# Roywangj/AdaptPoint

Measured on AMD Instinct MI355X. Metric: set-abstraction fwd+bwd point-clouds/sec (B=32,N=1024), higher is better.
Workload: dtype bf16

## Files before the change

### adaptpoint_amd/csrc/sa_fused.hip

```cpp
#include "apn_common.h"
#include "apn_mfma.h"
#include <type_traits>
#include "sa_chain.h"

namespace apn {

constexpr int SA_C = 32;
constexpr int SA_C1 = 32;
constexpr int SA_C2 = 64;
constexpr int SA_K = 32;
constexpr int SA_WAVES = 4;

template <int NS>
__device__ __forceinline__ void put_frag(uint4 *base, int f, int lane, const Frag<NS> &v) {
#pragma unroll
    for (int p = 0; p < NS; ++p) base[(f * NS + p) * 64 + lane] = __builtin_bit_cast(uint4, v.p[p]);
}

template <int NS>
__device__ __forceinline__ Frag<NS> get_frag(const uint4 *base, int f, int lane) {
    Frag<NS> v;
#pragma unroll
    for (int p = 0; p < NS; ++p) v.p[p] = __builtin_bit_cast(bf16x8, base[(f * NS + p) * 64 + lane]);
    return v;
// ... 292 lines not shown
    int nst = 3;
    for (; tile < tiles; slot += stride, tile = remap(slot)) {
        const bool more = remap(slot + stride) < tiles;
        const int tile2 = remap(slot + 2 * stride);
        if (LATE) {
            const TileHead hd_nxt2 = load_head<CP>(a, tile2 < tiles ? tile2 : tile, r);
            body(tile, cur, nst == 4, [&] {
                asm volatile("" ::: "memory");
                touch(hd_nxt);
                if (more) {
                    ahead(hd_nxt);
                    fetch_tile<NS>(a, hd_nxt, h, cur);
                }
            });
            stamp(a, wave, nst < 5 ? nst : 5);
            ++nst;
            hd_nxt = hd_nxt2;
            continue;
        }
        touch(hd_nxt);
        pre();
        if (more) fetch_tile<NS>(a, hd_nxt, h, nxt);
        const TileHead hd_nxt2 = load_head<CP>(a, tile2 < tiles ? tile2 : tile, r);
        body(tile, cur, nst == 4, [&] { touch(hd_nxt2); });
        stamp(a, wave, nst < 5 ? nst : 5);
        ++nst;
        if (more) cur = nxt;
        hd_nxt = hd_nxt2;
    }
    pre();
    stamp(a, wave, 6);
}

template <int NV>
__device__ __forceinline__ float fold_partials(float (&vals)[NV], int lane, int wave) {
    __shared__ float red[SA_WAVES][NV][32];
#pragma unroll
    for (int i = 0; i < NV; ++i) {
        const float other = __shfl_xor(vals[i], 32);
        if (lane < 32) red[wave][i][lane] = vals[i] + other;
    }
    __syncthreads();
    float s = 0.0f;
    const int e = threadIdx.x;
    if (e < NV * 32) {
#pragma unroll
        for (int w = 0; w < SA_WAVES; ++w) s += red[w][e >> 5][e & 31];
    }
    return s;
}

__device__ __forceinline__ void fold_rows32(const float *__restrict__ part, int rows, const double *__restrict__ sums,
                                            const BnArgs &bn, float *__restrict__ pack, float &scale, float &shift,
                                            double *scratch ) {
    double (*fred)[64] = reinterpret_cast<double (*)[64]>(scratch);
    double *ftot = scratch + 16 * 64;
    const int tid = threadIdx.x;
    double count = bn.count;
    double gpre = 1.0, bpre = 0.0;
    if (tid < 32) {
        if (bn.gamma) gpre = (double)bn.gamma[tid];
        if (bn.beta) bpre = (double)bn.beta[tid];
    }
    if (bn.training) {
        if (part) {
            const int quad = tid & 15, rg = tid >> 4;
            const float4 *__restrict__ p4 = reinterpret_cast<const float4 *>(part) + quad;
            double s0 = 0.0, s1 = 0.0, s2 = 0.0, s3 = 0.0;
            int rr = rg;
            for (; rr + 7 * 16 < rows; rr += 8 * 16) {
                float4 v[8];
#pragma unroll
                for (int u = 0; u < 8; ++u) v[u] = p4[(size_t)(rr + 16 * u) * 16];
#pragma unroll
                for (int u = 0; u < 8; ++u) {
                    s0 += (double)v[u].x; s1 += (double)v[u].y; s2 += (double)v[u].z; s3 += (double)v[u].w;
                }
            }
            for (; rr + 3 * 16 < rows; rr += 4 * 16) {
                float4 v[4];
#pragma unroll
                for (int u = 0; u < 4; ++u) v[u] = p4[(size_t)(rr + 16 * u) * 16];
#pragma unroll
                for (int u = 0; u < 4; ++u) {
                    s0 += (double)v[u].x; s1 += (double)v[u].y; s2 += (double)v[u].z; s3 += (double)v[u].w;
                }
            }
            for (; rr < rows; rr += 16) {
                const float4 v = p4[(size_t)rr * 16];
                s0 += (double)v.x; s1 += (double)v.y; s2 += (double)v.z; s3 += (double)v.w;
            }
            fred[rg][4 * quad] = s0; fred[rg][4 * quad + 1] = s1; fred[rg][4 * quad + 2] = s2; fred[rg][4 * quad + 3] = s3;
            __syncthreads();
            if (tid < 64) {
                double s = 0.0;
#pragma unroll
                for (int k = 0; k < 16; ++k) s += fred[k][tid];
                ftot[tid] = s;
            }
        } else if (tid < 64) {
            ftot[tid] = sums[tid];
        }
        if (!part) count = sums[64];
        __syncthreads();
    }
    if (tid < 32) {
        if (tid == 0 && blockIdx.x == 0 && bn.training && bn.nbt) *bn.nbt += 1;
        bn_channel(bn, 32, tid, bn.training ? ftot[tid] : 0.0, bn.training ? ftot[32 + tid] : 0.0, count,
                   blockIdx.x == 0, pack, scale, shift, gpre, bpre);
    }
}

template <int NS, bool CP>
__global__ __launch_bounds__(SA_WAVES * 64, 3) void sa_fwd_main_kernel(
    SaArgs a, const float *__restrict__ w2, BnArgs bn1, const float *__restrict__ part1, int rows1,
    const double *__restrict__ sums1, float *__restrict__ pack1, const float *__restrict__ gamma2,
    float *__restrict__ ysel, unsigned char *__restrict__ ksel, unsigned long long *__restrict__ acc2) {
    const int lane = threadIdx.x & 63, r = lane & 31, h = lane >> 5;
    const int wave = __builtin_amdgcn_readfirstlane(threadIdx.x >> 6);
    enum { F_W1 = 0, F_W2 = 3, F_COUNT = 7 };
    __shared__ uint4 cfrag[F_COUNT * NS * 64];
    __shared__ __attribute__((aligned(16))) float bn1v[2][2][16];
    constexpr int PT_WAVE = CP ? 2 * 32 * 33 : 17 * 64 * 2 / SA_WAVES;
    __shared__ __attribute__((aligned(16))) float ptile[SA_WAVES * PT_WAVE];
    __shared__ __attribute__((aligned(16))) unsigned sinfo[SA_WAVES][32];
    static_assert(SA_WAVES * PT_WAVE * 4 >= 17 * 64 * 8, "fold scratch");
    critical_stream_priority();
    stamp(a, wave, 0);
    const float sg[2] = {(!gamma2 || gamma2[r] >= 0.0f) ? 1.0f : -1.0f, (!gamma2 || gamma2[32 + r] >= 0.0f) ? 1.0f : -1.0f};
    float st[4] = {0.0f, 0.0f, 0.0f, 0.0f};

    auto prologue = [&]() {
        if (wave == 0) {
            Frag<NS> w1f[3];
            load_w1_frags<NS>(a.w1, r, h, w1f);
#pragma unroll
            for (int s = 0; s < 3; ++s) put_frag<NS>(cfrag, F_W1 + s, lane, w1f[s]);
        }
        if (wave == 1 || wave == 2) {
            const int t = wave - 1;
#pragma unroll
            for (int s = 0; s < 2; ++s) {
                float tmp[8];
#pragma unroll
                for (int j = 0; j < 8; ++j) tmp[j] = w2[(32 * t + r) * SA_C1 + acc_row(8 * s + j, h)];
                put_frag<NS>(cfrag, F_W2 + 2 * t + s, lane, make_frag<NS>(tmp));
            }
        }
        float sc, sh;
        fold_rows32(part1, rows1, sums1, bn1, pack1, sc, sh, reinterpret_cast<double *>(ptile));
        if (threadIdx.x < 32) {
            const int i = threadIdx.x;
            bn1v[0][(i >> 2) & 1][(i & 3) + 4 * (i >> 3)] = sc;
            bn1v[1][(i >> 2) & 1][(i & 3) + 4 * (i >> 3)] = sh;
        }
        __syncthreads();
    };

    for_each_tile<NS, CP>(a, wave, r, h, prologue, [] {}, [&](int tile, const TileRaw<NS> &raw, bool, auto before_stores) {
        int lane_o = lane;
        asm volatile("" : "+v"(lane_o));
        Frag<NS> x[3];
        build_frags<NS>(a, raw, h, x);
        const int q0 = __builtin_amdgcn_readfirstlane(raw.q0);
        const int nq = __builtin_amdgcn_readfirstlane((int)(raw.info >> 24));
        float multf[16];
        unsigned starts = 1u;
        float *pt = ptile + wave * PT_WAVE;
        if (CP) {
            if (lane < 32) sinfo[wave][lane] = raw.info;
#pragma unroll
            for (int gq = 0; gq < 4; ++gq) {
                const uint4 v = *reinterpret_cast<const uint4 *>(&sinfo[wave][8 * gq + 4 * (lane_o >> 5)]);
                multf[4 * gq] = (float)ri_mult(v.x); multf[4 * gq + 1] = (float)ri_mult(v.y);
                multf[4 * gq + 2] = (float)ri_mult(v.z); multf[4 * gq + 3] = (float)ri_mult(v.w);
            }
            const unsigned prev = (unsigned)__shfl_up((int)raw.info, 1);
            starts = (unsigned)__ballot(lane < 32 && (lane == 0 || ri_q(raw.info) != ri_q(prev)));
        }
        f32x16 y1 = {0};
#pragma unroll
        for (int s = 0; s < 3; ++s) y1 = mfma<NS>(get_frag<NS>(cfrag, F_W1 + s, lane_o), x[s], y1);
        {
            const float4 *scv = reinterpret_cast<const float4 *>(bn1v[0][lane_o >> 5]);
            const float4 *shv = reinterpret_cast<const float4 *>(bn1v[1][lane_o >> 5]);
#pragma unroll
            for (int i4 = 0; i4 < 4; ++i4) {
                const float4 sc = scv[i4], sh = shv[i4];
                y1[4 * i4] = __builtin_fmaxf(__builtin_fmaf(y1[4 * i4], sc.x, sh.x), 0.0f);
                y1[4 * i4 + 1] = __builtin_fmaxf(__builtin_fmaf(y1[4 * i4 + 1], sc.y, sh.y), 0.0f);
                y1[4 * i4 + 2] = __builtin_fmaxf(__builtin_fmaf(y1[4 * i4 + 2], sc.z, sh.z), 0.0f);
                y1[4 * i4 + 3] = __builtin_fmaxf(__builtin_fmaf(y1[4 * i4 + 3], sc.w, sh.w), 0.0f);
            }
        }
        const Frag<NS> a0 = pack8<NS>(y1, 0), a1 = pack8<NS>(y1, 8);
#pragma unroll
        for (int t = 0; t < 2; ++t) {
            f32x16 y2 = {0};
            y2 = mfma<NS>(a0, get_frag<NS>(cfrag, F_W2 + 2 * t, lane_o), y2);
            y2 = mfma<NS>(a1, get_frag<NS>(cfrag, F_W2 + 2 * t + 1, lane_o), y2);
            if (CP) {
                float s1 = 0.0f, s2 = 0.0f;
#pragma unroll
                for (int i = 0; i < 16; ++i) {
                    const float wy = multf[i] * y2[i];
                    s1 += wy;
                    s2 += wy * y2[i];
                    pt[(t * 32 + acc_row(i, h)) * 33 + r] = sg[t] * y2[i];
                }
                st[t] += s1;
                st[2 + t] += s2;
                continue;
            }
            float best = sg[t] * y2[0];
            int bpos = 0;
            float s1 = 0.0f, s2 = 0.0f;
#pragma unroll
            for (int i = 0; i < 16; ++i) {
                s1 += y2[i];
                s2 += y2[i] * y2[i];
                const float v = sg[t] * y2[i];
                if (i > 0 && v > best) { best = v; bpos = i; }
            }
            st[t] += s1;
            st[2 + t] += s2;
            int kpos = acc_row(bpos, h);
            const float obest = __shfl_xor(best, 32);
            const int okpos = __shfl_xor(kpos, 32);
            if (obest > best || (obest == best && okpos < kpos)) { best = obest; kpos = okpos; }
            if (h == 0) {
                ysel[(size_t)tile * SA_C2 + 32 * t + r] = sg[t] * best;
                ksel[(size_t)tile * SA_C2 + 32 * t + r] = (unsigned char)kpos;
            }
        }
        if (CP) {
            asm volatile("" ::: "memory");
            const float *mine = pt + h * (32 * 33) + r;
            const float sgn = h ? sg[1] : sg[0];
            float *ys = ysel + (size_t)q0 * SA_C2 + lane;
            unsigned char *ks = ksel + (size_t)q0 * SA_C2 + lane;
            before_stores();
            int seg = -1, ra = 0, kpos = 0;
            float best = 0.0f;
#pragma unroll
            for (int half16 = 0; half16 < 2; ++half16) {
                float v[16];
#pragma unroll
                for (int i = 0; i < 16; ++i) v[i] = mine[(16 * half16 + i) * 33];
#pragma unroll
                for (int i = 0; i < 16; ++i) {
                    const int rho = 16 * half16 + i;
                    if ((starts >> rho) & 1u) {
                        if (seg >= 0 && seg < nq) {
                            ys[(size_t)seg * SA_C2] = sgn * best;
                            ks[(size_t)seg * SA_C2] = (unsigned char)kpos;
                        }
                        ++seg;
                        best = -__builtin_inff();
                        kpos = 0;
                        ra = rho;
                    }
                    const bool up = v[i] > best;
                    best = up ? v[i] : best;
                    kpos = up ? rho - ra : kpos;
                }
            }
            if (seg >= 0 && seg < nq) {
                ys[(size_t)seg * SA_C2] = sgn * best;
                ks[(size_t)seg * SA_C2] = (unsigned char)kpos;
            }
            asm volatile("" ::: "memory");
        }
    });
    const float tot = fold_partials<4>(st, lane, wave);
    if (threadIdx.x < 128) acc_add(acc2, 128, blockIdx.x % ACC_COPIES, threadIdx.x, tot);
    stamp(a, wave, 7);
}

struct SaBwdArgs {
    const float *w2;
    const float *scale1, *shift1, *mean1, *inv1;
    const float *pack2;
    const unsigned long long *accS;
    const double *sumsS;
    double count;
    int train2;
    const float *goa;
    const unsigned char *ksel;
    const int *rowdst;
};

template <int NS, bool CP>
__global__ __launch_bounds__(SA_WAVES * 64, 2) void sa_bwd_kernel(SaArgs a, SaBwdArgs g,
                                                               unsigned long long *__restrict__ accT,
                                                               float *__restrict__ partW2,
                                                               float *__restrict__ GU,
                                                               float *__restrict__ HA,
                                                               float *__restrict__ HB) {
    static_assert(CP, "the backward pass runs over a tile map");
    const int lane = threadIdx.x & 63, r = lane & 31, h = lane >> 5;
    const int wave = __builtin_amdgcn_readfirstlane(threadIdx.x >> 6);
    enum { F_W1 = 0, F_QM = 3, F_W2T = 5, F_COUNT = 9 };
    __shared__ uint4 cfrag[F_COUNT * NS * 64];
    __shared__ __attribute__((aligned(16))) float bn1v[2][2][16];
    __shared__ __attribute__((aligned(16))) float sw2[SA_C2][SA_C1 + 4];
    __shared__ float sD[SA_C2], sE[SA_C2];
    __shared__ __attribute__((aligned(16))) float sqm[SA_C1 + 1][SA_C1 + 4];
    critical_stream_priority();
    stamp(a, wave, 0);
    __shared__ float chan[5][32];
    f32x16 dsp[2] = {{0}, {0}};
    f32x16 gram = {0};
    float suma = 0.0f;
    float st[2] = {0.0f, 0.0f};

    constexpr int SP_ROW = 72, SP_TILE = 32 * SP_ROW;
    constexpr int SP_WAVE = (CP && NS * SP_TILE * 2 < 2 * 32 * 33 * 4) ? 2 * 32 * 33 * 4 : NS * SP_TILE * 2;
    constexpr int SP_BYTES = SA_WAVES * SP_WAVE, WRED_BYTES = SA_WAVES * SA_C2 * SA_C1 * 4;
    __shared__ __attribute__((aligned(16))) unsigned char sp_raw[SP_BYTES > WRED_BYTES ? SP_BYTES : WRED_BYTES];
    __shared__ __attribute__((aligned(16))) unsigned sinfo[SA_WAVES][32];
    __shared__ __attribute__((aligned(16))) float qgoa[CP ? SA_WAVES : 1][4 * SA_C2];
    __shared__ __attribute__((aligned(16))) unsigned char qksel[CP ? SA_WAVES : 1][4 * SA_C2];
    __bf16 *sp_img = reinterpret_cast<__bf16 *>(sp_raw + wave * SP_WAVE);

    __shared__ __attribute__((aligned(16))) int sdst[SA_WAVES][2][64];
    int ahead_n = 0, body_n = 0;
    auto gu_store = [&](int place, float v) {
        *reinterpret_cast<float *>(reinterpret_cast<char *>(GU) + (((unsigned)place << 7) + ((unsigned)r << 2))) = v;
    };

    auto prologue = [&]() {
        const int tid = threadIdx.x;
        {
            Frag<NS> w1f[3];
            if (wave == 0) load_w1_frags<NS>(a.w1, r, h, w1f);
            float wv[8];
#pragma unroll
            for (int k = 0; k < 8; ++k) wv[k] = g.w2[tid + 256 * k];
            float c1[4] = {0.f, 0.f, 0.f, 0.f};
            if (tid >= 128 && tid < 160) {
                c1[0] = g.scale1[tid - 128]; c1[1] = g.shift1[tid - 128]; c1[2] = g.mean1[tid - 128]; c1[3] = g.inv1[tid - 128];
            }
            double sv = 0.0, count = g.count;
            float p_sc = 0.0f, p_mu = 0.0f, p_iv = 0.0f;
            if (tid < 128) sv = g.sumsS ? g.sumsS[tid] : acc_read(g.accS, 128, tid);
            if (g.sumsS) count = g.sumsS[128];
            if (tid < 64) { p_sc = g.pack2[tid]; p_mu = g.pack2[128 + tid]; p_iv = g.pack2[192 + tid]; }
            if (wave == 0) {
#pragma unroll
                for (int s = 0; s < 3; ++s) put_frag<NS>(cfrag, F_W1 + s, lane, w1f[s]);
            }
#pragma unroll
            for (int k = 0; k < 8; ++k) sw2[(tid + 256 * k) >> 5][tid & 31] = wv[k];
            if (tid >= 128 && tid < 160) {
#pragma unroll
                for (int k = 0; k < 4; ++k) chan[k][tid - 128] = c1[k];
            }
            double *sS2 = reinterpret_cast<double *>(&sqm[0][0]);
            if (tid >= 64 && tid < 128) sS2[tid - 64] = sv;
            __syncthreads();
            if (tid < 64) {
                const double sc = p_sc, mu = p_mu, iv = p_iv, s1 = sv, s2 = sS2[tid];
                double d = 0.0, e = 0.0;
                if (g.train2) {
                    const double rc = 1.0 / count;
                    d = -sc * iv * s2 * rc;
                    e = (-sc * s1 + sc * mu * iv * s2) * rc;
                }
                sD[tid] = (float)d;
                sE[tid] = (float)e;
            }
            if (tid >= 64 && tid < 96) {
                const int i = tid - 64;
                const float sci = g.scale1[i], shi = g.shift1[i];
                bn1v[0][(i >> 2) & 1][(i & 3) + 4 * (i >> 3)] = sci;
                bn1v[1][(i >> 2) & 1][(i & 3) + 4 * (i >> 3)] = shi;
            }
        }
        __syncthreads();
        {
            const int s = wave;
            float tmp[8], tmpd[8], tmpe[8];
#pragma unroll
            for (int j = 0; j < 8; ++j) {
                const int c = 16 * s + 8 * h + j;
                tmp[j] = sw2[c][r];
                tmpd[j] = tmp[j] * sD[c];
                tmpe[j] = r == 0 ? sE[c] : 0.0f;
            }
            const Frag<NS> wt = make_frag<NS>(tmp);
            put_frag<NS>(cfrag, F_W2T + s, lane, wt);
            const f32x16 zero16 = {0};
            const f32x16 qp = mfma<NS>(make_frag<NS>(tmpd), wt, zero16);
            const f32x16 ep = mfma<NS>(make_frag<NS>(tmpe), wt, zero16);
            float *scr = reinterpret_cast<float *>(sp_img);
#pragma unroll
            for (int e = 0; e < 16; ++e) scr[e * 64 + lane] = qp[e];
            if (h == 0) scr[16 * 64 + r] = ep[0];
        }
        __syncthreads();
        if (wave == 2) {
            f32x16 qacc = {0};
            float ev = 0.0f;
#pragma unroll
            for (int w = 0; w < SA_WAVES; ++w) {
                const float *pw = reinterpret_cast<const float *>(sp_raw + w * SP_WAVE);
#pragma unroll
                for (int e = 0; e < 16; ++e) qacc[e] += pw[e * 64 + lane];
                if (h == 0) ev += pw[16 * 64 + r];
            }
            put_frag<NS>(cfrag, F_QM, lane, pack8<NS>(qacc, 0));
            put_frag<NS>(cfrag, F_QM + 1, lane, pack8<NS>(qacc, 8));
            if (h == 0) chan[4][r] = ev;
        }
        __syncthreads();
        {
            uint4 *z = reinterpret_cast<uint4 *>(sp_img);
            for (int e = lane; e < SP_WAVE / 16; e += 64) z[e] = make_uint4(0u, 0u, 0u, 0u);
        }
    };

    auto scatter_pending = [] {};
    auto ahead = [&](const TileHead &hd) {
        if (!CP) return;
        typedef __attribute__((address_space(3))) void lds_void;
        typedef __attribute__((address_space(1))) const void glb_void;
        const int q0n = __builtin_amdgcn_readfirstlane(hd.q0);
        const int qbn = q0n < a.b * a.m - 4 ? q0n : a.b * a.m - 4;
        int l_o = lane;
        asm volatile("" : "+v"(l_o));
        const char *gb = reinterpret_cast<const char *>(g.goa) + (size_t)qbn * (SA_C2 * 4);
        const char *kb = reinterpret_cast<const char *>(g.ksel) + (size_t)qbn * SA_C2;
        __builtin_amdgcn_global_load_lds((glb_void *)(gb + (unsigned)(16 * l_o)), (lds_void *)&qgoa[wave][0], 16, 0, 0);
        __builtin_amdgcn_global_load_lds((glb_void *)(kb + (unsigned)(4 * l_o)), (lds_void *)&qksel[wave][0], 4, 0, 0);
        const char *db = reinterpret_cast<const char *>(g.rowdst) + (size_t)__builtin_amdgcn_readfirstlane(hd.tile) * (SA_K * 4);
        __builtin_amdgcn_global_load_lds((glb_void *)(db + (unsigned)(4 * (l_o & 31))), (lds_void *)&sdst[wave][ahead_n & 1][0], 4, 0, 0);
        ++ahead_n;
    };
    for_each_tile<NS, CP, CP>(a, wave, r, h, prologue, scatter_pending, [&](int tile, const TileRaw<NS> &raw, bool probe, auto before_stores) {
        auto st2 = [&](int k) { if (probe) stamp(a, wave, 8 + k); };
        st2(0);
        int lane_o = lane;
        asm volatile("" : "+v"(lane_o));
        Frag<NS> x[3];
        build_frags<NS>(a, raw, h, x);

        const int q0 = __builtin_amdgcn_readfirstlane(raw.q0);
        const int nq = CP ? __builtin_amdgcn_readfirstlane((int)(raw.info >> 24)) : 1;
        const bool live_row = !CP || ri_mult(raw.info) != 0;
        const float mrow = CP ? (float)ri_mult(raw.info) : 1.0f;
        float gv4[4];
        int kc4[4];
        const int qb = q0 < a.b * a.m - 4 ? q0 : a.b * a.m - 4;
#pragma unroll
        for (int u = 0; u < 4; ++u) {
            if (CP) {
                gv4[u] = 0.0f;
                kc4[u] = 0;
            } else {
                gv4[u] = 0.0f;
                kc4[u] = 0;
                if (u == 0) {
                    gv4[u] = g.goa[(size_t)(q0 + u) * SA_C2 + lane];
                    kc4[u] = g.ksel[(size_t)(q0 + u) * SA_C2 + lane];
                }
            }
        }
        unsigned mpk[4] = {0x01010101u, 0x01010101u, 0x01010101u, 0x01010101u};
        unsigned starts = 1u;
        if (CP) {
            if (lane < 32) sinfo[wave][lane] = raw.info;
#pragma unroll
            for (int gq = 0; gq < 4; ++gq) {
                const uint4 v = *reinterpret_cast<const uint4 *>(&sinfo[wave][8 * gq + 4 * (lane_o >> 5)]);
                mpk[gq] = ri_mult(v.x) | (ri_mult(v.y) << 8) | (ri_mult(v.z) << 16) | (ri_mult(v.w) << 24);
            }
            const unsigned prev = (unsigned)__shfl_up((int)raw.info, 1);
            starts = (unsigned)__ballot(lane < 32 && (lane == 0 || ri_q(raw.info) != ri_q(prev)));
        }
        auto multf = [&](int i) { return (float)((mpk[i >> 2] >> (8 * (i & 3))) & 0xffu); };
        f32x16 yT = {0}, y1 = {0};
#pragma unroll
        for (int s = 0; s < 3; ++s) {
            const Frag<NS> w = get_frag<NS>(cfrag, F_W1 + s, lane_o);
            yT = mfma<NS>(w, x[s], yT);
            y1 = mfma<NS>(x[s], w, y1);
        }
        {
            const float4 *scv = reinterpret_cast<const float4 *>(bn1v[0][lane_o >> 5]);
            const float4 *shv = reinterpret_cast<const float4 *>(bn1v[1][lane_o >> 5]);
#pragma unroll
            for (int i4 = 0; i4 < 4; ++i4) {
                const float4 sc = scv[i4], sh = shv[i4];
                yT[4 * i4] = __builtin_fmaxf(__builtin_fmaf(yT[4 * i4], sc.x, sh.x), 0.0f);
                yT[4 * i4 + 1] = __builtin_fmaxf(__builtin_fmaf(yT[4 * i4 + 1], sc.y, sh.y), 0.0f);
                yT[4 * i4 + 2] = __builtin_fmaxf(__builtin_fmaf(yT[4 * i4 + 2], sc.z, sh.z), 0.0f);
                yT[4 * i4 + 3] = __builtin_fmaxf(__builtin_fmaf(yT[4 * i4 + 3], sc.w, sh.w), 0.0f);
            }
        }
        st2(1);
        Frag<NS> a0, a1;
        if (CP) {
            f32x16 yw;
#pragma unroll
            for (int i = 0; i < 16; ++i) yw[i] = yT[i] * mrow;
            a0 = pack8<NS>(yw, 0);
            a1 = pack8<NS>(yw, 8);
        } else {
            a0 = pack8<NS>(yT, 0);
            a1 = pack8<NS>(yT, 8);
        }

        Frag<NS> sp[4];
        {
            unsigned todo = starts;
            if (CP) {
                asm volatile("s_waitcnt vmcnt(0)" ::: "memory");
                const int dq = q0 - qb;
#pragma unroll
                for (int u = 0; u < 4; ++u) {
                    const int e = (u + dq < 4 ? u + dq : 3) * SA_C2 + lane_o;
                    gv4[u] = qgoa[wave][e];
                    kc4[u] = qksel[wave][e];
                }
            }
#pragma unroll 1
            for (int jb = 0; jb < nq; jb += 4) {
                if (jb) {
#pragma unroll
                    for (int u = 0; u < 4; ++u)
                        if (jb + u < nq) {
                            gv4[u] = g.goa[(size_t)(q0 + jb + u) * SA_C2 + lane];
                            kc4[u] = g.ksel[(size_t)(q0 + jb + u) * SA_C2 + lane];
                        }
                }
#pragma unroll
                for (int u = 0; u < 4; ++u) {
                    if (jb + u < nq) {
                        const float gv = gv4[u];
                        int kc = kc4[u];
                        if (CP) {
                            kc += __builtin_ctz(todo);
                            todo &= todo - 1u;
                        }
                        const __bf16 ghi = (__bf16)gv;
                        const __bf16 glo = (__bf16)(gv - (float)ghi);
                        __bf16 *cell = sp_img + kc * SP_ROW + lane;
                        cell[0] = ghi;
                        if (NS == 2) cell[SP_TILE] = glo;
                        if (!CP) kc4[u] = kc;
                    }
                }
            }
        }
        asm volatile("" ::: "memory");
        {
            f32x16 an;
            const float sc1 = chan[0][lane_o & 31], sh1 = chan[1][lane_o & 31];
#pragma unroll
            for (int i = 0; i < 16; ++i) {
                an[i] = __builtin_fmaxf(__builtin_fmaf(y1[i], sc1, sh1), 0.0f);
                if (CP) suma = __builtin_fmaf(multf(i), an[i], suma);
                else suma += an[i];
            }
            const Frag<NS> b0 = pack8<NS>(an, 0), b1 = pack8<NS>(an, 8);
            if (CP) {
                f32x16 aw;
#pragma unroll
                for (int i = 0; i < 16; ++i) aw[i] = an[i] * multf(i);
                gram = mfma<NS>(pack8<NS>(aw, 0), b0, gram);
                gram = mfma<NS>(pack8<NS>(aw, 8), b1, gram);
            } else {
                gram = mfma<NS>(b0, b0, gram);
                gram = mfma<NS>(b1, b1, gram);
            }
            typedef short tr_s4 __attribute__((ext_vector_type(4)));
            typedef short tr_s8 __attribute__((ext_vector_type(8)));
            typedef __attribute__((address_space(3))) tr_s4 tr_lds;
            const int li = lane_o & 15, gq = li >> 2, gp = li & 3, grh = (lane_o >> 4) & 1;
            const __bf16 *tb = sp_img + (4 * (lane_o >> 5) + gq) * SP_ROW + 16 * grh + 4 * gp;
#pragma unroll
            for (int t = 0; t < 2; ++t) {
#pragma unroll
                for (int sk = 0; sk < 2; ++sk) {
                    Frag<NS> at;
#pragma unroll
                    for (int pp = 0; pp < NS; ++pp) {
                        const __bf16 *src = tb + pp * SP_TILE + (16 * sk) * SP_ROW + 32 * t;
                        const tr_s4 lo4 = __builtin_amdgcn_ds_read_tr16_b64_v4i16((tr_lds *)(src));
                        const tr_s4 hi4 = __builtin_amdgcn_ds_read_tr16_b64_v4i16((tr_lds *)(src + 8 * SP_ROW));
                        const tr_s8 v8 = {lo4.x, lo4.y, lo4.z, lo4.w, hi4.x, hi4.y, hi4.z, hi4.w};
                        at.p[pp] = __builtin_bit_cast(bf16x8, v8);
                    }
                    dsp[t] = mfma<NS>(at, sk ? b1 : b0, dsp[t]);
                }
            }
        }
        st2(2);
#pragma unroll
        for (int s = 0; s < 4; ++s) {
            const __bf16 *src = sp_img + r * SP_ROW + 16 * s + 8 * h;
            sp[s].p[0] = *reinterpret_cast<const bf16x8 *>(src);
            if (NS == 2) sp[s].p[NS - 1] = *reinterpret_cast<const bf16x8 *>(src + SP_TILE);
        }
        asm volatile("" ::: "memory");
        if (!CP) {
            __bf16 *cell = sp_img + kc4[0] * SP_ROW + lane;
            cell[0] = (__bf16)0.0f;
            if (NS == 2) cell[SP_TILE] = (__bf16)0.0f;
        }
        f32x16 ga;
        const float ev = chan[4][lane_o & 31];
#pragma unroll
        for (int i = 0; i < 16; ++i) ga[i] = CP ? ev * multf(i) : ev;
        ga = mfma<NS>(a0, get_frag<NS>(cfrag, F_QM, lane_o), ga);
        ga = mfma<NS>(a1, get_frag<NS>(cfrag, F_QM + 1, lane_o), ga);
#pragma unroll
        for (int s = 0; s < 4; ++s) ga = mfma<NS>(sp[s], get_frag<NS>(cfrag, F_W2T + s, lane_o), ga);

        st2(3);
        float *gt = reinterpret_cast<float *>(sp_img);
        asm volatile("" ::: "memory");
        float s1 = 0.0f, s2 = 0.0f, hb = 0.0f;
        const float sc1l = chan[0][lane_o & 31], sh1l = chan[1][lane_o & 31], iv1 = chan[3][lane_o & 31];
        const float nmi = -chan[2][lane_o & 31] * iv1;
#pragma unroll
        for (int i = 0; i < 16; ++i) {
            const float u = __builtin_fmaf(y1[i], sc1l, sh1l);
            const float yhat = __builtin_fmaf(y1[i], iv1, nmi);
            ga[i] = u > 0.0f ? ga[i] : 0.0f;
            s1 += ga[i];
            s2 += ga[i] * yhat;
            if (CP) {
                gt[acc_row(i, h) * 33 + r] = ga[i];
                gt[32 * 33 + acc_row(i, h) * 33 + r] = multf(i) * yhat;
            } else {
                hb += yhat;
            }
        }
        st[0] += s1;
        st[1] += s2;

        st2(4);
        before_stores();
        {
            int live;
            if (CP) {
                asm volatile("" ::: "memory");
                const float *mine = gt + h * (32 * 33) + r;
                float *dst = (h ? HB : HA) + (size_t)q0 * SA_C1 + r;
                int seg = -1;
                float sum = 0.0f;
#pragma unroll
                for (int half16 = 0; half16 < 2; ++half16) {
                    float v[16];
#pragma unroll
                    for (int i = 0; i < 16; ++i) v[i] = mine[(16 * half16 + i) * 33];
#pragma unroll
                    for (int i = 0; i < 16; ++i) {
                        if ((starts >> (16 * half16 + i)) & 1u) {
                            if (seg >= 0 && seg < nq) dst[(size_t)seg * SA_C1] = sum;
                            ++seg;
                            sum = 0.0f;
                        }
                        sum += v[i];
                    }
                }
                if (seg >= 0 && seg < nq) dst[(size_t)seg * SA_C1] = sum;
                asm volatile("" ::: "memory");
                {
                    uint4 *z = reinterpret_cast<uint4 *>(sp_img);
#pragma unroll
                    for (int e = 0; e < (NS * SP_TILE * 2 / 16 + 63) / 64; ++e)
                        if (e * 64 + lane < NS * SP_TILE * 2 / 16) z[e * 64 + lane] = make_uint4(0u, 0u, 0u, 0u);
                }
                asm volatile("" ::: "memory");
                live = __popcll(__ballot(lane < 32 && live_row));
            } else {
                const float ha = s1 + __shfl_xor(s1, 32);
                hb += __shfl_xor(hb, 32);
                if (h == 0) {
                    HA[(size_t)tile * SA_C1 + r] = ha;
                    HB[(size_t)tile * SA_C1 + r] = hb;
                }
                live = 0;
            }

            st2(5);
            st2(6);
            if (CP) {
                const int *dl = &sdst[wave][body_n & 1][0];
#pragma unroll
                for (int gq = 0; gq < 4; ++gq) {
                    if (8 * gq < live) {
                        const int4 dd = *reinterpret_cast<const int4 *>(&dl[8 * gq + 4 * (lane_o >> 5)]);
                        const int base = 8 * gq + 4 * h;
                        if (base + 0 < live) gu_store(dd.x, ga[4 * gq + 0]);
                        if (base + 1 < live) gu_store(dd.y, ga[4 * gq + 1]);
                        if (base + 2 < live) gu_store(dd.z, ga[4 * gq + 2]);
                        if (base + 3 < live) gu_store(dd.w, ga[4 * gq + 3]);
                    }
                }
            }
            ++body_n;
        }
    }, ahead);
    {
        const float tot = fold_partials<2>(st, lane, wave);
        if (threadIdx.x < 64) acc_add(accT, 64, blockIdx.x % ACC_COPIES, threadIdx.x, tot);
    }
    float (*wred)[SA_C2 * SA_C1] = reinterpret_cast<float (*)[SA_C2 * SA_C1]>(sp_raw);
    __syncthreads();
#pragma unroll
    for (int i = 0; i < 16; ++i) {
        wred[wave][acc_row(i, h) * SA_C1 + r] = dsp[0][i];
        wred[wave][(32 + acc_row(i, h)) * SA_C1 + r] = dsp[1][i];
    }
    __syncthreads();
    const int ec = threadIdx.x >> 2, emid = (threadIdx.x & 3) * 8;
    float sp8[8];
    {
        float4 lo4 = make_float4(0.f, 0.f, 0.f, 0.f), hi4 = lo4;
#pragma unroll
        for (int w = 0; w < SA_WAVES; ++w) {
            const float4 a4 = *reinterpret_cast<const float4 *>(&wred[w][ec * SA_C1 + emid]);
            const float4 b4 = *reinterpret_cast<const float4 *>(&wred[w][ec * SA_C1 + emid + 4]);
            lo4.x += a4.x; lo4.y += a4.y; lo4.z += a4.z; lo4.w += a4.w;
            hi4.x += b4.x; hi4.y += b4.y; hi4.z += b4.z; hi4.w += b4.w;
        }
        sp8[0] = lo4.x; sp8[1] = lo4.y; sp8[2] = lo4.z; sp8[3] = lo4.w;
        sp8[4] = hi4.x; sp8[5] = hi4.y; sp8[6] = hi4.z; sp8[7] = hi4.w;
    }
    __syncthreads();
    suma += __shfl_xor(suma, 32);
#pragma unroll
    for (int i = 0; i < 16; ++i) wred[wave][acc_row(i, h) * SA_C1 + r] = gram[i];
    if (h == 0) wred[wave][SA_C1 * SA_C1 + r] = suma;
    __syncthreads();
    for (int e = threadIdx.x; e < SA_C1 * SA_C1 + SA_C1; e += SA_WAVES * 64)
        sqm[e >> 5][e & 31] = (wred[0][e] + wred[1][e]) + (wred[2][e] + wred[3][e]);
    __syncthreads();
    {
        float acc[8];
#pragma unroll
        for (int j = 0; j < 8; ++j) acc[j] = 0.0f;
#pragma unroll 8
        for (int k = 0; k < SA_C1; ++k) {
            const float w = sw2[ec][k];
            const float4 g0 = *reinterpret_cast<const float4 *>(&sqm[k][emid]);
            const float4 g1 = *reinterpret_cast<const float4 *>(&sqm[k][emid + 4]);
            acc[0] = __builtin_fmaf(w, g0.x, acc[0]); acc[1] = __builtin_fmaf(w, g0.y, acc[1]);
            acc[2] = __builtin_fmaf(w, g0.z, acc[2]); acc[3] = __builtin_fmaf(w, g0.w, acc[3]);
            acc[4] = __builtin_fmaf(w, g1.x, acc[4]); acc[5] = __builtin_fmaf(w, g1.y, acc[5]);
            acc[6] = __builtin_fmaf(w, g1.z, acc[6]); acc[7] = __builtin_fmaf(w, g1.w, acc[7]);
        }
        const float d = sD[ec], e = sE[ec];
        const float4 s0 = *reinterpret_cast<const float4 *>(&sqm[32][emid]);
        const float4 s1 = *reinterpret_cast<const float4 *>(&sqm[32][emid + 4]);
        float4 *row = reinterpret_cast<float4 *>(partW2 + (size_t)blockIdx.x * (SA_C2 * SA_C1) + ec * SA_C1 + emid);
        row[0] = make_float4(sp8[0] + d * acc[0] + e * s0.x, sp8[1] + d * acc[1] + e * s0.y,
                             sp8[2] + d * acc[2] + e * s0.z, sp8[3] + d * acc[3] + e * s0.w);
        row[1] = make_float4(sp8[4] + d * acc[4] + e * s1.x, sp8[5] + d * acc[5] + e * s1.y,
                             sp8[6] + d * acc[6] + e * s1.z, sp8[7] + d * acc[7] + e * s1.w);
    }
    stamp(a, wave, 7);
}

static int sa_grid(int tiles, bool compact = false) {
    const int cap = compact ? 768 : 512;
    int g = (tiles + SA_WAVES - 1) / SA_WAVES;
    return g < cap ? (g < 1 ? 1 : g) : cap;
}

static int sa_grid_bwd(int tiles) {
    int g = sa_grid(tiles);
    return g < 448 ? g : 448;
}

}

extern "C" int apn_sa_grid_blocks(int b, int m) { return apn::sa_grid(b * m); }
extern "C" int apn_sa_grid_rows(int b, int m, int with_tile_map) { return apn::sa_grid(b * m, with_tile_map != 0); }
extern "C" int apn_sa_bwd_main_rows(int b, int m) { return apn::sa_grid_bwd(b * m); }
extern "C" int apn_sa_acc_words(int ncol) { return ncol > 0 ? apn::acc_words(ncol) : 0; }

extern "C" int apn_sa_prep_rows(int b, int n) {
    const long long tiles = (long long)b * ((n + apn::PS_PTS - 1) / apn::PS_PTS);
    return (int)(tiles < apn::PS_MAX_ROWS ? (tiles < 1 ? 1 : tiles) : apn::PS_MAX_ROWS);
}

extern "C" int apn_sa_prep_stats(int b, int n, const float *f, const void *geo, const void *dd, const float *w1,
                                 int precision, int stats, void *ft, float *part1, void *zero, long long zero_words,
                                 void *stream) {
    using namespace apn;
    if (b <= 0 || n <= 0 || b > 65535 || (precision != 1 && precision != 2) || !f || !ft || !w1) return APN_EINVAL;
    if (stats && (!geo || !dd || !part1 || ((uintptr_t)geo & 15) || ((uintptr_t)part1 & 15))) return APN_EINVAL;
    if (zero_words < 0 || (zero_words && !zero)) return APN_EINVAL;
    __bf16 *hi = (__bf16 *)ft;
    __bf16 *lo = precision == 2 ? hi + (size_t)b * n * SA_C : nullptr;
    const int tpc = (n + PS_PTS - 1) / PS_PTS;
    auto kern = precision == 2 ? sa_prep_stats_kernel<2> : sa_prep_stats_kernel<1>;
    const int lds = SA_C * (PS_PTS + 1) * (int)sizeof(float);
    static DynLdsOnce lds_set[2];
    if (hipError_t e = set_dyn_lds(lds_set[precision - 1], (const void *)kern, lds)) return (int)e;
    hipLaunchKernelGGL(kern, dim3(apn_sa_prep_rows(b, n)), dim3(PS_NT), lds, (hipStream_t)stream, n, tpc, b * tpc, f,
                       (const long long *)geo, (const double *)dd, b * (apn_sa_geo_dd_doubles(n) / 6), w1, stats, hi, lo, part1,
                       (unsigned long long *)zero, zero_words);
    APN_LAUNCH_CHECK();
    return APN_OK;
}

#ifdef APN_WG_STAMPS
extern "C" __attribute__((visibility("default"))) int apn_sa_debug_wg_stamps_fused(void *buf) {
    return (int)hipMemcpyToSymbol(HIP_SYMBOL(apn::d_wg_stamps_f), &buf, sizeof(buf));
}
#endif

static unsigned long long *g_stamps = nullptr;
extern "C" int apn_sa_debug_stamps(void *buf) { g_stamps = (unsigned long long *)buf; return APN_OK; }

static apn::SaArgs sa_args(int b, int n, int m, const float *xyz, const float *new_xyz, const void *ft,
                           int precision, const int *idx, const float *w1, float radius, const int *tmap) {
    const __bf16 *hi = (const __bf16 *)ft;
    return apn::SaArgs{b, n, m, xyz, new_xyz, hi,
                       precision == 2 ? hi + (size_t)b * n * apn::SA_C : nullptr, idx, w1, radius, tmap, g_stamps};
}

static int sa_check(int b, int n, int m, int precision) {
    if (precision != 1 && precision != 2) return APN_EINVAL;
    if (b <= 0 || n <= 0 || m <= 0) return APN_EINVAL;
    if ((long long)b * m > 0x7fffffffLL / 64) return APN_EINVAL;
    if ((long long)b * n > 0xffffffffLL / 256) return APN_EINVAL;
    if ((long long)b * m > 0xffffffffLL / (32 * 128)) return APN_EINVAL;
    return APN_OK;
}

extern "C" int apn_sa_fwd_main(int b, int n, int m, int precision, float radius, const float *xyz,
                               const float *new_xyz, const void *ft, const int *idx, const int *tmap, const float *w1,
                               const float *w2, const float *g1, const float *b1, float *rm1, float *rv1, void *nbt1,
                               float eps1, float mom1, int train1, double count, const float *part1, int rows1,
                               const double *sums1, float *pack1, const float *gamma2, float *ysel, void *ksel,
                               void *acc2, void *stream) {
    using namespace apn;
    if (int e = sa_check(b, n, m, precision)) return e;
    if (!xyz || !new_xyz || !ft || !idx || !w1 || !w2 || !pack1 || !ysel || !ksel || !acc2) return APN_EINVAL;
    if (train1 && !part1 && !sums1) return APN_EINVAL;
    if (!train1 && (!rm1 || !rv1)) return APN_EINVAL;
    if (part1 && (((uintptr_t)part1 & 15) || rows1 <= 0)) return APN_EINVAL;
    SaArgs a = sa_args(b, n, m, xyz, new_xyz, ft, precision, idx, w1, radius, tmap);
    BnArgs bn{g1, b1, rm1, rv1, (long long *)nbt1, eps1, mom1, train1, count};
    auto kern = precision == 2 ? (tmap ? sa_fwd_main_kernel<2, true> : sa_fwd_main_kernel<2, false>)
                               : (tmap ? sa_fwd_main_kernel<1, true> : sa_fwd_main_kernel<1, false>);
    hipLaunchKernelGGL(kern, dim3(sa_grid(b * m, tmap != nullptr)), dim3(SA_WAVES * 64), 0, (hipStream_t)stream, a, w2, bn,
                       sums1 ? nullptr : part1, rows1, sums1, pack1, gamma2, ysel, (unsigned char *)ksel,
                       (unsigned long long *)acc2);
    APN_LAUNCH_CHECK();
    return APN_OK;
}

extern "C" int apn_sa_bwd_main(int b, int n, int m, int precision, float radius, const float *xyz,
                               const float *new_xyz, const void *ft, const int *idx, const int *tmap, const float *w1,
                               const float *w2, const float *pack1, const float *pack2, const void *accS,
                               const double *sumsS, double count, int train2, const float *goa, const void *ksel,
                               void *accT, float *partW2, const int *rowdst, float *GU, float *HA, float *HB, void *stream) {
    using namespace apn;
    if (int e = sa_check(b, n, m, precision)) return e;
    if (!w2 || !pack1 || !pack2 || (!accS && !sumsS) || !goa || !ksel || !accT || !partW2 || !GU || !HA || !HB)
        return APN_EINVAL;
    if (!tmap || !rowdst) return APN_EINVAL;
    SaArgs a = sa_args(b, n, m, xyz, new_xyz, ft, precision, idx, w1, radius, tmap);
    SaBwdArgs g;
    g.w2 = w2;
    g.scale1 = pack1; g.shift1 = pack1 + 32; g.mean1 = pack1 + 64; g.inv1 = pack1 + 96;
    g.pack2 = pack2;
    g.accS = (const unsigned long long *)accS; g.sumsS = sumsS;
    g.count = count; g.train2 = train2;
    g.goa = goa; g.ksel = (const unsigned char *)ksel;
    g.rowdst = rowdst;
    auto kern = precision == 2 ? sa_bwd_kernel<2, true> : sa_bwd_kernel<1, true>;
    hipLaunchKernelGGL(kern, dim3(sa_grid_bwd(b * m)), dim3(SA_WAVES * 64), 0, (hipStream_t)stream, a, g,
                       (unsigned long long *)accT, partW2, GU, HA, HB);
    APN_LAUNCH_CHECK();
    return APN_OK;
}
```

Measured before the change: 121,100.

## Reuse gram operand via LDS transpose instead of recomputing transposed layer-1 product

Result: no change. 120,900 (-0.2%).

```diff
diff --git a/adaptpoint_amd/csrc/sa_fused.hip b/adaptpoint_amd/csrc/sa_fused.hip
--- a/adaptpoint_amd/csrc/sa_fused.hip
+++ b/adaptpoint_amd/csrc/sa_fused.hip
@@ -618,7 +618,6 @@
     const int wave = __builtin_amdgcn_readfirstlane(threadIdx.x >> 6);
     enum { F_W1 = 0, F_QM = 3, F_W2T = 5, F_COUNT = 9 };
     __shared__ uint4 cfrag[F_COUNT * NS * 64];
-    __shared__ __attribute__((aligned(16))) float bn1v[2][2][16];
     __shared__ __attribute__((aligned(16))) float sw2[SA_C2][SA_C1 + 4];
     __shared__ float sD[SA_C2], sE[SA_C2];
     __shared__ __attribute__((aligned(16))) float sqm[SA_C1 + 1][SA_C1 + 4];
@@ -641,8 +640,8 @@
 
     __shared__ __attribute__((aligned(16))) int sdst[SA_WAVES][2][64];
     int ahead_n = 0, body_n = 0;
-    auto gu_store = [&](int place, float v) {
-        *reinterpret_cast<float *>(reinterpret_cast<char *>(GU) + (((unsigned)place << 7) + ((unsigned)r << 2))) = v;
+    auto gu_store = [&](int place, int mid, float v) {
+        *reinterpret_cast<float *>(reinterpret_cast<char *>(GU) + (((unsigned)place << 7) + ((unsigned)mid << 2))) = v;
     };
 
     auto prologue = [&]() {
@@ -685,12 +684,6 @@
                 }
                 sD[tid] = (float)d;
                 sE[tid] = (float)e;
-            }
-            if (tid >= 64 && tid < 96) {
-                const int i = tid - 64;
-                const float sci = g.scale1[i], shi = g.shift1[i];
-                bn1v[0][(i >> 2) & 1][(i & 3) + 4 * (i >> 3)] = sci;
-                bn1v[1][(i >> 2) & 1][(i & 3) + 4 * (i >> 3)] = shi;
             }
         }
         __syncthreads();
@@ -764,7 +757,6 @@
         const int q0 = __builtin_amdgcn_readfirstlane(raw.q0);
         const int nq = CP ? __builtin_amdgcn_readfirstlane((int)(raw.info >> 24)) : 1;
         const bool live_row = !CP || ri_mult(raw.info) != 0;
-        const float mrow = CP ? (float)ri_mult(raw.info) : 1.0f;
         float gv4[4];
         int kc4[4];
         const int qb = q0 < a.b * a.m - 4 ? q0 : a.b * a.m - 4;
@@ -784,6 +776,7 @@
         }
         unsigned mpk[4] = {0x01010101u, 0x01010101u, 0x01010101u, 0x01010101u};
         unsigned starts = 1u;
+        auto repack = [&] { asm volatile("" : "+v"(mpk[0]), "+v"(mpk[1]), "+v"(mpk[2]), "+v"(mpk[3])); };
         if (CP) {
             if (lane < 32) sinfo[wave][lane] = raw.info;
 #pragma unroll
@@ -791,43 +784,16 @@
                 const uint4 v = *reinterpret_cast<const uint4 *>(&sinfo[wave][8 * gq + 4 * (lane_o >> 5)]);
                 mpk[gq] = ri_mult(v.x) | (ri_mult(v.y) << 8) | (ri_mult(v.z) << 16) | (ri_mult(v.w) << 24);
             }
+            repack();
             const unsigned prev = (unsigned)__shfl_up((int)raw.info, 1);
             starts = (unsigned)__ballot(lane < 32 && (lane == 0 || ri_q(raw.info) != ri_q(prev)));
         }
         auto multf = [&](int i) { return (float)((mpk[i >> 2] >> (8 * (i & 3))) & 0xffu); };
-        f32x16 yT = {0}, y1 = {0};
-#pragma unroll
-        for (int s = 0; s < 3; ++s) {
-            const Frag<NS> w = get_frag<NS>(cfrag, F_W1 + s, lane_o);
-            yT = mfma<NS>(w, x[s], yT);
-            y1 = mfma<NS>(x[s], w, y1);
-        }
-        {
-            const float4 *scv = reinterpret_cast<const float4 *>(bn1v[0][lane_o >> 5]);
-            const float4 *shv = reinterpret_cast<const float4 *>(bn1v[1][lane_o >> 5]);
-#pragma unroll
-            for (int i4 = 0; i4 < 4; ++i4) {
-                const float4 sc = scv[i4], sh = shv[i4];
-                yT[4 * i4] = __builtin_fmaxf(__builtin_fmaf(yT[4 * i4], sc.x, sh.x), 0.0f);
-                yT[4 * i4 + 1] = __builtin_fmaxf(__builtin_fmaf(yT[4 * i4 + 1], sc.y, sh.y), 0.0f);
-                yT[4 * i4 + 2] = __builtin_fmaxf(__builtin_fmaf(yT[4 * i4 + 2], sc.z, sh.z), 0.0f);
-                yT[4 * i4 + 3] = __builtin_fmaxf(__builtin_fmaf(yT[4 * i4 + 3], sc.w, sh.w), 0.0f);
-            }
-        }
+        f32x16 y1 = {0};
+#pragma unroll
+        for (int s = 0; s < 3; ++s) y1 = mfma<NS>(x[s], get_frag<NS>(cfrag, F_W1 + s, lane_o), y1);
         st2(1);
-        Frag<NS> a0, a1;
-        if (CP) {
-            f32x16 yw;
-#pragma unroll
-            for (int i = 0; i < 16; ++i) yw[i] = yT[i] * mrow;
-            a0 = pack8<NS>(yw, 0);
-            a1 = pack8<NS>(yw, 8);
-        } else {
-            a0 = pack8<NS>(yT, 0);
-            a1 = pack8<NS>(yT, 8);
-        }
-
-        Frag<NS> sp[4];
+
         {
             unsigned todo = starts;
             if (CP) {
@@ -870,6 +836,7 @@
             }
         }
         asm volatile("" ::: "memory");
+        Frag<NS> awf[2];
         {
             f32x16 an;
             const float sc1 = chan[0][lane_o & 31], sh1 = chan[1][lane_o & 31];
@@ -879,17 +846,20 @@
                 if (CP) suma = __builtin_fmaf(multf(i), an[i], suma);
                 else suma += an[i];
             }
+            asm volatile("" : "+v"(suma));
             const Frag<NS> b0 = pack8<NS>(an, 0), b1 = pack8<NS>(an, 8);
             if (CP) {
                 f32x16 aw;
 #pragma unroll
                 for (int i = 0; i < 16; ++i) aw[i] = an[i] * multf(i);
-                gram = mfma<NS>(pack8<NS>(aw, 0), b0, gram);
-                gram = mfma<NS>(pack8<NS>(aw, 8), b1, gram);
+                awf[0] = pack8<NS>(aw, 0);
+                awf[1] = pack8<NS>(aw, 8);
             } else {
-                gram = mfma<NS>(b0, b0, gram);
-                gram = mfma<NS>(b1, b1, gram);
-            }
+                awf[0] = b0;
+                awf[1] = b1;
+            }
+            gram = mfma<NS>(awf[0], b0, gram);
+            gram = mfma<NS>(awf[1], b1, gram);
             typedef short tr_s4 __attribute__((ext_vector_type(4)));
             typedef short tr_s8 __attribute__((ext_vector_type(8)));
             typedef __attribute__((address_space(3))) tr_s4 tr_lds;
@@ -913,11 +883,14 @@
             }
         }
         st2(2);
+        f32x16 ga = {0};
 #pragma unroll
         for (int s = 0; s < 4; ++s) {
             const __bf16 *src = sp_img + r * SP_ROW + 16 * s + 8 * h;
-            sp[s].p[0] = *reinterpret_cast<const bf16x8 *>(src);
-            if (NS == 2) sp[s].p[NS - 1] = *reinterpret_cast<const bf16x8 *>(src + SP_TILE);
+            Frag<NS> sps;
+            sps.p[0] = *reinterpret_cast<const bf16x8 *>(src);
+            if (NS == 2) sps.p[NS - 1] = *reinterpret_cast<const bf16x8 *>(src + SP_TILE);
+            ga = mfma<NS>(sps, get_frag<NS>(cfrag, F_W2T + s, lane_o), ga);
         }
         asm volatile("" ::: "memory");
         if (!CP) {
@@ -925,14 +898,45 @@
             cell[0] = (__bf16)0.0f;
             if (NS == 2) cell[SP_TILE] = (__bf16)0.0f;
         }
-        f32x16 ga;
-        const float ev = chan[4][lane_o & 31];
-#pragma unroll
-        for (int i = 0; i < 16; ++i) ga[i] = CP ? ev * multf(i) : ev;
+        Frag<NS> a0, a1;
+        {
+            typedef short tr_s4 __attribute__((ext_vector_type(4)));
+            typedef short tr_s8 __attribute__((ext_vector_type(8)));
+            typedef __attribute__((address_space(3))) tr_s4 tr_lds;
+            constexpr int T_PART = 32 * 32 * 2;
+            static_assert(NS * T_PART <= SP_WAVE, "the transposed operand is staged in the image's region");
+            unsigned char *stg = reinterpret_cast<unsigned char *>(sp_img);
+            const unsigned lo_ = (unsigned)lane_o, hh = lo_ >> 5;
+            const unsigned wb = ((lo_ & 31u) << 6) + ((hh ^ ((lo_ >> 2) & 7u)) << 3);
+#pragma unroll
+            for (int s = 0; s < 2; ++s) {
+#pragma unroll
+                for (int pp = 0; pp < NS; ++pp) {
+                    const uint4 v = __builtin_bit_cast(uint4, awf[s].p[pp]);
+                    *reinterpret_cast<uint2 *>(stg + pp * T_PART + (wb ^ (unsigned)(32 * s))) = make_uint2(v.x, v.y);
+                    *reinterpret_cast<uint2 *>(stg + pp * T_PART + (wb ^ (unsigned)(32 * s + 16))) = make_uint2(v.z, v.w);
+                }
+            }
+            asm volatile("" ::: "memory");
+            const unsigned li = lo_ & 15u, gq = li >> 2, gp = li & 3u, grh = (lo_ >> 4) & 1u;
+            const unsigned rb = ((4u * hh + gq) << 6) + (((4u * grh + gp) ^ hh) << 3);
+#pragma unroll
+            for (int s = 0; s < 2; ++s) {
+                Frag<NS> at;
+#pragma unroll
+                for (int pp = 0; pp < NS; ++pp) {
+                    const unsigned char *src = stg + pp * T_PART + 1024 * s;
+                    const tr_s4 lo4 = __builtin_amdgcn_ds_read_tr16_b64_v4i16((tr_lds *)(src + (rb ^ (unsigned)(32 * s))));
+                    const tr_s4 hi4 = __builtin_amdgcn_ds_read_tr16_b64_v4i16((tr_lds *)(src + 512 + (rb ^ (unsigned)(32 * s + 16))));
+                    const tr_s8 v8 = {lo4.x, lo4.y, lo4.z, lo4.w, hi4.x, hi4.y, hi4.z, hi4.w};
+                    at.p[pp] = __builtin_bit_cast(bf16x8, v8);
+                }
+                if (s) a1 = at; else a0 = at;
+            }
+            asm volatile("" ::: "memory");
+        }
         ga = mfma<NS>(a0, get_frag<NS>(cfrag, F_QM, lane_o), ga);
         ga = mfma<NS>(a1, get_frag<NS>(cfrag, F_QM + 1, lane_o), ga);
-#pragma unroll
-        for (int s = 0; s < 4; ++s) ga = mfma<NS>(sp[s], get_frag<NS>(cfrag, F_W2T + s, lane_o), ga);
 
         st2(3);
         float *gt = reinterpret_cast<float *>(sp_img);
@@ -940,11 +944,13 @@
         float s1 = 0.0f, s2 = 0.0f, hb = 0.0f;
         const float sc1l = chan[0][lane_o & 31], sh1l = chan[1][lane_o & 31], iv1 = chan[3][lane_o & 31];
         const float nmi = -chan[2][lane_o & 31] * iv1;
+        const float ev = chan[4][lane_o & 31];
+        if (CP) repack();
 #pragma unroll
         for (int i = 0; i < 16; ++i) {
             const float u = __builtin_fmaf(y1[i], sc1l, sh1l);
             const float yhat = __builtin_fmaf(y1[i], iv1, nmi);
-            ga[i] = u > 0.0f ? ga[i] : 0.0f;
+            ga[i] = u > 0.0f ? __builtin_fmaf(ev, CP ? multf(i) : 1.0f, ga[i]) : 0.0f;
             s1 += ga[i];
             s2 += ga[i] * yhat;
             if (CP) {
@@ -959,13 +965,14 @@
 
         st2(4);
         before_stores();
+        int lane_t = lane;
+        asm volatile("" : "+v"(lane_t));
         {
             int live;
             if (CP) {
                 asm volatile("" ::: "memory");
-                const float *mine = gt + h * (32 * 33) + r;
-                float *dst = (h ? HB : HA) + (size_t)q0 * SA_C1 + r;
-                int seg = -1;
+                float *mine = gt + (lane_t >> 5) * (32 * 33) + (lane_t & 31);
+                float *dst = ((lane_t >> 5) ? HB : HA) + (size_t)q0 * SA_C1 + (lane_t & 31);
                 float sum = 0.0f;
 #pragma unroll
                 for (int half16 = 0; half16 < 2; ++half16) {
@@ -974,21 +981,36 @@
                     for (int i = 0; i < 16; ++i) v[i] = mine[(16 * half16 + i) * 33];
 #pragma unroll
                     for (int i = 0; i < 16; ++i) {
-                        if ((starts >> (16 * half16 + i)) & 1u) {
-                            if (seg >= 0 && seg < nq) dst[(size_t)seg * SA_C1] = sum;
-                            ++seg;
-                            sum = 0.0f;
-                        }
-                        sum += v[i];
+                        const float keep = __builtin_bit_cast(float, (((starts >> (16 * half16 + i)) & 1u) - 1u) & 0x3f800000u);
+                        sum = __builtin_fmaf(sum, keep, v[i]);
+                        mine[(16 * half16 + i) * 33] = sum;
                     }
                 }
-                if (seg >= 0 && seg < nq) dst[(size_t)seg * SA_C1] = sum;
+                unsigned rest = starts;
+                float tot[4];
+#pragma unroll
+                for (int u = 0; u < 4; ++u) {
+                    rest &= rest - 1u;
+                    const int last = rest ? __builtin_ctz(rest) - 1 : 31;
+                    tot[u] = mine[last * 33];
+                }
+#pragma unroll
+                for (int u = 0; u < 4; ++u)
+                    if (u < nq) dst[u * SA_C1] = tot[u];
+#pragma unroll 1
+                for (int u = 4; u < nq; ++u) {
+                    rest &= rest - 1u;
+                    const int last = rest ? __builtin_ctz(rest) - 1 : 31;
+                    dst[(size_t)u * SA_C1] = mine[last * 33];
+                }
                 asm volatile("" ::: "memory");
                 {
                     uint4 *z = reinterpret_cast<uint4 *>(sp_img);
+                    unsigned z0 = 0u;
+                    asm volatile("" : "+v"(z0));
 #pragma unroll
                     for (int e = 0; e < (NS * SP_TILE * 2 / 16 + 63) / 64; ++e)
-                        if (e * 64 + lane < NS * SP_TILE * 2 / 16) z[e * 64 + lane] = make_uint4(0u, 0u, 0u, 0u);
+                        if (e * 64 + lane_t < NS * SP_TILE * 2 / 16) z[e * 64 + lane_t] = make_uint4(z0, z0, z0, z0);
                 }
                 asm volatile("" ::: "memory");
                 live = __popcll(__ballot(lane < 32 && live_row));
@@ -1009,12 +1031,12 @@
 #pragma unroll
                 for (int gq = 0; gq < 4; ++gq) {
                     if (8 * gq < live) {
-                        const int4 dd = *reinterpret_cast<const int4 *>(&dl[8 * gq + 4 * (lane_o >> 5)]);
-                        const int base = 8 * gq + 4 * h;
-                        if (base + 0 < live) gu_store(dd.x, ga[4 * gq + 0]);
-                        if (base + 1 < live) gu_store(dd.y, ga[4 * gq + 1]);
-                        if (base + 2 < live) gu_store(dd.z, ga[4 * gq + 2]);
-                        if (base + 3 < live) gu_store(dd.w, ga[4 * gq + 3]);
+                        const int4 dd = *reinterpret_cast<const int4 *>(&dl[8 * gq + 4 * (lane_t >> 5)]);
+                        const int base = 8 * gq + 4 * (lane_t >> 5), mid = lane_t & 31;
+                        if (base + 0 < live) gu_store(dd.x, mid, ga[4 * gq + 0]);
+                        if (base + 1 < live) gu_store(dd.y, mid, ga[4 * gq + 1]);
+                        if (base + 2 < live) gu_store(dd.z, mid, ga[4 * gq + 2]);
+                        if (base + 3 < live) gu_store(dd.w, mid, ga[4 * gq + 3]);
                     }
                 }
             }
```
